# dcmlr/groundgrid

Measured on AMD Instinct MI355X. Metric: point clouds/s (Velodyne-64, ~120k pts, 120m/0.33m grid), higher is better.
Workload: dtype f32+f64 (the reference's mixed float/double arithmetic, bit-exact)

## Files before the change

groundgrid_amd/csrc/gg_context.hip:

```cpp
#include <float.h>
#include <math.h>
#include <stdio.h>
#include <string.h>

#include <algorithm>
#include <atomic>
#include <condition_variable>
#include <cstdlib>
#include <cstdio>
#include <functional>
#include <mutex>
#include <string>
#include <thread>
#include <tuple>
#include <vector>
#include <chrono>

#include <dlfcn.h>
#include <sched.h>
#include <unistd.h>

#include "gg_internal.h"
#include "arena_layout.h"
#include "hip_owned.h"
#include "host_helper.h"
#include "plane_args.h"
#include "region_args.h"
#include "scroll_core.h"
#include "sweep_core.h"

using namespace gg;

namespace {

constexpr int EXPORT_VARIANT_DEFAULT = 0;
constexpr int IMPORT_VARIANT_DEFAULT = 0;
constexpr int IMAGES_VARIANT_DEFAULT = 0;
constexpr int K_SCORE = GG_NUM_KERNELS;

struct EventPair {
    hipEvent_t start, stop;
    int kernel;
    bool owns_start;
};

struct ParamRing {
    Event done[PARAM_RING], done2[PARAM_RING];
    bool used[PARAM_RING]{}, used2[PARAM_RING]{};
    int next = 0;
    hipError_t create()
    {
        hipError_t e = hipSuccess;
        for (int i = 0; i < PARAM_RING && e == hipSuccess; ++i) e = done[i].create();
        for (int i = 0; i < PARAM_RING && e == hipSuccess; ++i) e = done2[i].create();
        return e;
    }
    hipError_t acquire(int *g)
    {
        *g = next;
        next = (next + 1) % PARAM_RING;
        hipError_t e = used[*g] ? hipEventSynchronize(done[*g]) : hipSuccess;
        if (e == hipSuccess && used2[*g]) e = hipEventSynchronize(done2[*g]);
        if (e == hipSuccess) used[*g] = used2[*g] = false;
        return e;
    }
    hipError_t recorded(int g, hipStream_t st)
    {
        const hipError_t e = hipEventRecord(done[g], st);
        if (e == hipSuccess) used[g] = true;
        return e;
    }
    hipError_t recorded2(int g, hipStream_t half_stream)
    {
        const hipError_t e = hipEventRecord(done2[g], half_stream);
        if (e == hipSuccess) used2[g] = true;
        return e;
    }
};

struct CallScratch {
    DeviceBlock<char> dev;
    PinnedBlock<char> pinned;
};

struct RingPart {
    size_t dev, pinned, per_entry;
};
template <typename T>
struct RingTable {
    T *host = nullptr, *dev = nullptr;
    size_t per_entry = 0;
    void bind(const CallScratch &m, const RingPart &p)
    {
        host = (T *)(m.pinned + p.pinned);
        dev = (T *)(m.dev + p.dev);
        per_entry = p.per_entry;
// ... 520 lines not shown
    {
        StageRange stage("interpolation");
        sweep::Params sp = ctx->sweep_params;
        sp.decrease = ctx->cfg.occupied_cells_decrease_factor;
        sp.inv_decrease = 1.0 / sp.decrease;
        sp.decay_fast = sp.decrease >= 1.25 && sp.decrease < 1e300;
        launch_sweep(a, sp, dp, nb, s, ctx->d_sweep_dbg);
    }
    prof.end();
    {
        StageRange stage("segmentation");
        prof.begin(GG_K_LABEL);
        launch_label(a, dp, io, nb, max_n, s);
        prof.end();
        if (score) {
            prof.begin(K_SCORE);
            launch_score(a, dp, io, ctx->score, nb, max_n, s);
            prof.end();
        }
    }
    if (side) hipStreamWaitEvent(s, ctx->join_event, 0);
}

void drop_graphs(gg_context *ctx)
{
    for (auto &e : ctx->graphs) {
        if (e.exec) hipGraphExecDestroy(e.exec);
        if (e.graph) hipGraphDestroy(e.graph);
    }
    ctx->graphs.clear();
}

int launch_or_replay(gg_context *ctx, const Arena &a, const CloudParams *hp, CloudParams *dp, const BatchIO &io, int nb, int max_n, hipStream_t s, const LayerPlan *plan,
                     bool score)
{
    const bool profile = (ctx->flags & GG_FLAG_PROFILE) != 0;
    const bool eligible = nb == 1 && !plan && ctx->graphs_enabled && !profile && !ctx->d_sweep_dbg && s != nullptr && !a.k2_debug && !a.k3_debug && !a.k5_debug && !a.k2_skip;
    if (!eligible) {
        HIPCHK(ctx, hipMemcpyAsync(dp, hp, sizeof(CloudParams) * nb, hipMemcpyHostToDevice, s));
        launch_sequence(ctx, a, dp, io, nb, max_n, s, plan, hp[0].slot, profile, score);
        return GG_OK;
    }
    gg_context::GraphKey key;
    memset(&key, 0, sizeof key);
    key.io = io;
    key.max_n = (int)std::min(ctx->max_points, io.cloud_stride);
    key.slot = hp[0].slot;
    key.flags = a.flags;
    key.eigen = a.eigen_reduction;
    key.generation = ctx->graph_generation;
    key.stream = s;
    if (plan) {
        key.layer_mask = plan->mask & EARLY_LAYERS;
        for (int l = 0; l < GG_NUM_LAYERS; ++l) key.layer_dst[l] = ((key.layer_mask >> l) & 1u) ? plan->dst[l] : nullptr;
    }
    gg_context::GraphEntry *entry = nullptr;
    for (auto &e : ctx->graphs)
        if (memcmp(&e.key, &key, sizeof key) == 0) entry = &e;
    if (!entry) {
        if (ctx->graphs.size() >= 8) {
            size_t victim = 0;
            for (size_t k = 1; k < ctx->graphs.size(); ++k)
                if (ctx->graphs[k].last_use < ctx->graphs[victim].last_use) victim = k;
            if (ctx->graphs[victim].exec) hipGraphExecDestroy(ctx->graphs[victim].exec);
            if (ctx->graphs[victim].graph) hipGraphDestroy(ctx->graphs[victim].graph);
            ctx->graphs.erase(ctx->graphs.begin() + (long)victim);
        }
        ctx->graphs.emplace_back();
        entry = &ctx->graphs.back();
        entry->key = key;
    }
    entry->last_use = ++ctx->graph_clock;
// ... 58 lines not shown
{
    const bool lazy = (ctx->flags & GG_FLAG_MINIMAL_LAYERS) || (batch_entry && !(ctx->flags & GG_FLAG_EAGER_LAYERS));
    const unsigned eff_flags = lazy ? (ctx->flags | GG_FLAG_MINIMAL_LAYERS) : (ctx->flags & ~(unsigned)GG_FLAG_MINIMAL_LAYERS);
    const int nb = b->n_clouds;
    if (nb == 0) return GG_OK;
    int g;
    HIPCHK(ctx, ctx->ring.acquire(&g));
    CloudParams *hp = ctx->h_params + (size_t)g * ctx->n_slots;
    CloudParams *dp = ctx->d_params + (size_t)g * ctx->n_slots;
    int n_first = nb;
    const bool split_wanted = halves_enabled(ctx) && !plan && nb >= ctx->halves_min_clouds && s != ctx->half_stream && s != nullptr;
    if (split_wanted) {
        n_first = 0;
        for (int i = 0; i < nb; ++i) n_first += second_half_slot(ctx, slot_of(b->slots, b->first_slot, i)) ? 0 : 1;
    }
    const bool split = split_wanted && n_first > 0 && n_first < nb;
    if (!split) n_first = nb;
    int max_n[2] = {0, 0}, at[2] = {0, n_first};
    for (int i = 0; i < nb; ++i) {
        const int slot = slot_of(b->slots, b->first_slot, i);
        const int half = split && second_half_slot(ctx, slot) ? 1 : 0;
        CloudParams &p = hp[at[half]++];
        p.slot = slot;
        p.n_points = b->n_points[i];
        p.ox = b->origins[i * 3 + 0];
        p.oy = b->origins[i * 3 + 1];
        p.oz = b->origins[i * 3 + 2];
        p.base_z = (float)b->base_z[i];
        p.pos_x = ctx->pos_x[slot];
        p.pos_y = ctx->pos_y[slot];
        p.has_tf = b->transforms ? 1 : 0;
        p.no_confidence = ctx->no_confidence[slot] ? 1 : 0;
        p.fresh = 0;
        ctx->no_confidence[slot] = 0;
        for (int k = 0; k < 12; ++k) p.tf[k] = b->transforms ? b->transforms[(size_t)i * 12 + k] : 0.0;
        p.label_shift = nb == 1 ? ctx->next_label_shift : 0;
        p.io_index = i;
        p.cfg_index = ctx->slot_own[slot] ? slot : -1;
        if (!confidences_stay_positive(ctx->slot_own[slot] ? ctx->slot_cfg[slot] : ctx->cfg)) ctx->gp_tainted[slot] = 1;
        max_n[half] = std::max(max_n[half], p.n_points);
        ctx->lazy_pending[slot] = lazy ? 1 : 0;
        if (lazy) ctx->lazy_params[slot] = p;
    }
    bool score_half[2] = {false, false};
    if (ctx->score_n_ids)
        for (int i = 0; i < nb; ++i) score_half[i < n_first ? 0 : 1] |= ctx->score_on[hp[i].slot] != 0;
    const bool own_masks = (score_half[0] || score_half[1]) && !b->d_label_masks;
    bool fresh_half[2] = {false, false};
    for (int h = 0; h < (split ? 2 : 1); ++h) {
        const int lo = h ? n_first : 0, hi = h ? nb : n_first;
        bool all = ctx->fresh_enabled && !plan && !ctx->d_sweep_dbg && sweep_takes_fresh(ctx->arena, ctx->sweep_params, hi - lo);
        for (int i = lo; i < hi && all; ++i) all = ctx->fresh[hp[i].slot] != 0 && !ctx->gp_tainted[hp[i].slot];
        fresh_half[h] = all;
        if (all)
            for (int i = lo; i < hi; ++i) hp[i].fresh = 1, ctx->fresh[hp[i].slot] = 0;
    }
    auto fill_fresh = [&](int lo, int hi, hipStream_t on) -> int {
        for (int i = lo; i < hi;) {
            int e = i + 1;
            while (e < hi && hp[e].slot == hp[e - 1].slot + 1) ++e;
            if (const int rc = make_real(ctx, hp[i].slot, e - i, on)) return rc;
            i = e;
        }
        return GG_OK;
    };
    if (s != ctx->stream && ctx->map_event_pending) HIPCHK(ctx, hipStreamWaitEvent(s, ctx->map_event, 0));
    if (ctx->have_batch_event && ctx->last_batch_stream != s && !ctx->probe_unordered_streams) HIPCHK(ctx, hipStreamWaitEvent(s, ctx->batch_event, 0));
    bool joined = false;
    if (!(split && ctx->last_batch_stream == s)) {
        if (const int rc = stream_waits_for_second_half(ctx, s)) return rc;
        joined = true;
    }
    if (split) {
        gg_context::HalvesRecord now;
        const size_t per = b->cloud_stride;
        const uint8_t *p6[7] = {(const uint8_t *)b->d_labels, (const uint8_t *)b->d_out_index, (const uint8_t *)b->d_out_clouds, (const uint8_t *)b->d_out_counts,
                                (const uint8_t *)b->d_label_masks, (const uint8_t *)b->d_out_pc2, own_masks ? ctx->d_score_masks : nullptr};
        const size_t bytes6[7] = {(size_t)nb * per, (size_t)nb * per * 4, (size_t)nb * per * sizeof(gg_point32), (size_t)nb * 64, (size_t)nb * ((per + 3) / 4), (size_t)nb * per * 18,
                                  (size_t)nb * ((per + 3) / 4)};
        for (int k = 0; k < 7; ++k) now.lo[k] = p6[k], now.hi[k] = p6[k] ? p6[k] + bytes6[k] : nullptr;
        uint64_t h = 1469598103934665603ull;
        for (int i = 0; i < nb; ++i) h = (h ^ (uint64_t)(second_half_slot(ctx, slot_of(b->slots, b->first_slot, i)) ? 2 * i + 1 : 2 * i)) * 1099511628211ull;
        now.map_hash = h ^ (uint64_t)nb;
        bool clash = false;
        for (int r = 0; r < ctx->halves_hist_n && !joined && !clash; ++r) {
            const gg_context::HalvesRecord &o = ctx->halves_hist[r];
            if (o.map_hash == now.map_hash) continue;
            for (int x = 0; x < 7 && !clash; ++x)
// ... 26 lines not shown
    io.cloud_stride = b->cloud_stride;
    io.point_format = b->point_format;
    io.d_labels = b->d_labels;
    io.d_out_index = b->d_out_index;
    io.d_out_clouds = b->d_out_clouds;
    io.d_out_counts = b->d_out_counts;
    io.d_label_masks = b->d_label_masks;
    io.d_out_pc2 = b->d_out_pc2;
    BatchIO io_score = io;
    if (own_masks) io_score.d_label_masks = ctx->d_score_masks;

    Arena a = ctx->arena;
    a.flags = eff_flags;
    a.eigen_reduction = ctx->conv.eigen_reduction;
    a.fresh_launch = 0;
    bool own_half[2] = {false, false};
    for (int i = 0; i < nb; ++i) own_half[i < n_first ? 0 : 1] |= hp[i].cfg_index >= 0;
    a.slot_cfg_launch = own_half[0] ? 1 : 0;
    if (split) {
        if (!ctx->probe_no_fork) {
            HIPCHK(ctx, hipEventRecord(ctx->half_fork, s));
            HIPCHK(ctx, hipStreamWaitEvent(ctx->half_stream, ctx->half_fork, 0));
        }
        Arena a2 = a;
        a2.front_sync = a.front_sync2;
        a2.sweep_sync = a.sweep_sync2;
        a2.sweep_rec_clouds = 0;
        a2.scan_sync = a.scan_sync2;
        a2.slot_cfg_launch = own_half[1] ? 1 : 0;
        a.fresh_launch = fresh_half[0] ? 1 : 0;
        a2.fresh_launch = fresh_half[1] ? 1 : 0;
        if (const int rc = fill_fresh(0, n_first, s)) return rc;
        if (const int rc = fill_fresh(n_first, nb, ctx->half_stream)) return rc;
        HIPCHK(ctx, hipMemcpyAsync(dp, hp, sizeof(CloudParams) * n_first, hipMemcpyHostToDevice, s));
        HIPCHK(ctx, hipMemcpyAsync(dp + n_first, hp + n_first, sizeof(CloudParams) * (nb - n_first), hipMemcpyHostToDevice, ctx->half_stream));
        launch_sequence(ctx, a, dp, score_half[0] ? io_score : io, n_first, max_n[0], s, nullptr, hp[0].slot, false, score_half[0]);
        launch_sequence(ctx, a2, dp + n_first, score_half[1] ? io_score : io, nb - n_first, max_n[1], ctx->half_stream, nullptr, hp[n_first].slot, false, score_half[1]);
        HIPCHK(ctx, hipGetLastError());
        HIPCHK(ctx, ctx->ring.recorded2(g, ctx->half_stream));
        HIPCHK(ctx, hipEventRecord(ctx->half_done, ctx->half_stream));
        ctx->have_half_event = true;
    } else {
        a.fresh_launch = fresh_half[0] ? 1 : 0;
        if (const int rc = fill_fresh(0, nb, s)) return rc;
        if (const int rc = launch_or_replay(ctx, a, hp, dp, score_half[0] ? io_score : io, nb, max_n[0], s, plan, score_half[0])) return rc;
        HIPCHK(ctx, hipGetLastError());
    }
    HIPCHK(ctx, ctx->ring.recorded(g, s));
    HIPCHK(ctx, hipEventRecord(ctx->batch_event, s));
    ctx->last_batch_stream = s;
    ctx->have_batch_event = true;
    if (s != ctx->stream) ctx->map_event_pending = false;
    return GG_OK;
}

struct TableUpload {
    size_t offset;
    const void *src;
    size_t bytes;
};
int alloc_call_scratch(gg_context *ctx, const char *who, hipStream_t st, size_t dev_bytes, size_t pinned_bytes, std::initializer_list<TableUpload> tables, CallScratch *mem,
                       ParamRing *ring)
{
    hipStreamCaptureStatus cs = hipStreamCaptureStatusNone;
    if (hipStreamIsCapturing(st, &cs) == hipSuccess && cs != hipStreamCaptureStatusNone)
        return fail(ctx, GG_ERR_INVALID, who, "the first call allocates its scratch and cannot be captured into a graph");
    (void)hipGetLastError();
    CallScratch m;
    ParamRing r;
    int code = GG_ERR_NOMEM;
    const char *what = "device scratch";
    hipError_t e = m.dev.create(dev_bytes);
    if (e == hipSuccess) {
        what = "pinned parameter ring";
        e = m.pinned.create(pinned_bytes);
    }
    if (e == hipSuccess) code = GG_ERR_HIP;
    if (e == hipSuccess && ring) {
// ... 628 lines not shown
        out12[r * 4 + 3] = pose7[r];
    }
    return GG_OK;
}

int gg_get_size(const gg_context *ctx, int *rows, int *cols)
{
    if (!ctx) return GG_ERR_INVALID;
    if (rows) *rows = ctx->arena.g.rows;
    if (cols) *cols = ctx->arena.g.cols;
    return GG_OK;
}

int gg_get_geometry(const gg_context *ctx, double *resolution, double *length_x, double *length_y)
{
    if (!ctx) return GG_ERR_INVALID;
    if (resolution) *resolution = ctx->arena.g.resolution;
    if (length_x) *length_x = ctx->arena.g.length0;
    if (length_y) *length_y = ctx->arena.g.length1;
    return GG_OK;
}

const char *gg_last_error(const gg_context *ctx) { return ctx ? ctx->last_error.c_str() : "null context"; }

int gg_reset_maps(gg_context *ctx, int first_slot, int n, double pos_x, double pos_y, float odom_z, int persistent_only, void *stream)
{
    if (!ctx) return GG_ERR_INVALID;
    if (n < 0) return fail(ctx, GG_ERR_CAPACITY, "gg_reset_maps: n < 0");
    if (const int rc = check_slot_list(ctx, "gg_reset_maps", n, nullptr, first_slot)) return rc;
    if (n == 0) return GG_OK;
    HIPCHK(ctx, hipSetDevice(ctx->device));
    const hipStream_t st = pick_stream(ctx, stream);
    for (int s = first_slot; s < first_slot + n; ++s) ctx->fresh[s] = 0;
    const int boundary = (ctx->n_slots + 1) / 2;
    const bool split = halves_enabled(ctx) && st != ctx->stream && st != ctx->half_stream && st != nullptr && first_slot < boundary && first_slot + n > boundary;
    if (const int rc = call_follows_context(ctx, st, split)) return rc;
    const Arena &a = ctx->arena;
    for (int s = first_slot; s < first_slot + n; ++s) {
        ctx->no_confidence[s] = 1;
        ctx->pos_x[s] = pos_x;
        ctx->pos_y[s] = pos_y;
    }
    const float init[GG_NUM_LAYERS] = {0.0f, odom_z, (float)0.0000001, (float)100.0, (float)-100.0, 0.f, 0.f, 0.f, 0.f, 0.f, 0.f};
    auto fill = [&](int first, int count, hipStream_t on) {
        if (count <= 0) return;
        if (!persistent_only) {
            for (int s = first; s < first + count; ++s) ctx->lazy_pending[s] = 0;
            launch_fill_percall(a, first, count, init, on);
            launch_fill_bytes((uint8_t *)(a.tile_live + (size_t)first * a.tile_live_stride), (size_t)count * a.tile_live_stride * 4, 0xFF, on);
        }
        if (ctx->fresh_enabled) {
            for (int s = first; s < first + count;) {
                if (!ctx->gp_tainted[s]) {
                    ++s;
                    continue;
                }
                int e = s + 1;
                while (e < first + count && ctx->gp_tainted[e]) ++e;
                launch_fill2_strided(gp2_ptr(a, s), (size_t)a.gpl.elems, a.gp2_stride, e - s, init[GG_LAYER_GROUND], init[GG_LAYER_GROUNDPATCH], a.gp_valid, on);
                for (int k = s; k < e; ++k) ctx->gp_tainted[k] = 0;
                s = e;
            }
            launch_reset_fresh(a, first, count, init[GG_LAYER_GROUND], init[GG_LAYER_GROUNDPATCH], on);
            for (int s = first; s < first + count; ++s) ctx->fresh[s] = 1, ctx->fresh_z[s] = odom_z;
        } else {
            launch_fill2_strided(gp2_ptr(a, first), (size_t)a.gpl.elems, a.gp2_stride, count, init[GG_LAYER_GROUND], init[GG_LAYER_GROUNDPATCH], a.gp_valid, on);
            for (int s = first; s < first + count; ++s) ctx->gp_tainted[s] = 0;
        }
    };
    if (split) {
        if (!ctx->probe_no_fork) {
            HIPCHK(ctx, hipEventRecord(ctx->half_fork, st));
            HIPCHK(ctx, hipStreamWaitEvent(ctx->half_stream, ctx->half_fork, 0));
        }
        fill(first_slot, boundary - first_slot, st);
        fill(boundary, first_slot + n - boundary, ctx->half_stream);
        HIPCHK(ctx, hipGetLastError());
        HIPCHK(ctx, hipEventRecord(ctx->half_done, ctx->half_stream));
        ctx->have_half_event = true;
    } else {
        fill(first_slot, n, st);
        HIPCHK(ctx, hipGetLastError());
    }
    return call_recorded(ctx, st, false);
}

int gg_reset_map(gg_context *ctx, int slot, double pos_x, double pos_y, float odom_z)
{
    if (!slot_ok(ctx, slot)) return GG_ERR_CAPACITY;
    return gg_reset_maps(ctx, slot, 1, pos_x, pos_y, odom_z, 0, nullptr);
}

int gg_set_map_position(gg_context *ctx, int slot, double pos_x, double pos_y)
{
    if (!slot_ok(ctx, slot)) return GG_ERR_CAPACITY;
    ctx->pos_x[slot] = pos_x;
// ... 2304 lines not shown
```

groundgrid_amd/csrc/gg_internal.h:

```cpp
#pragma once

#include <hip/hip_runtime.h>
#include <stdint.h>

#include <atomic>
#include <mutex>

#include "groundgrid_hip.h"
#include "gp_layout.h"

namespace gg {

constexpr int TILE = 16;
constexpr int TILE_CELLS = TILE * TILE;
constexpr uint32_t KEY_OUTSIDE = 0xFFFFFFFFu;
constexpr int K2_DBG_WGS = 32768;
constexpr int PW_BIG_CONTEXT_SLOTS = 128;
constexpr int SWEEP_LATENCY_MAX_CLOUDS = 256;
constexpr int K2_MIN_GROUPS_PER_CLOUD = 64;
constexpr int PACKED_TILE_COUNTERS_MIN_T = 1024;
constexpr int K2_LIGHT_MAX = 512;
constexpr int KEY_TILE_SHIFT = 12;
constexpr int SCAN_MAX_PARTS = 16, SCAN_SYNC_WORDS = 1 + SCAN_MAX_PARTS;
constexpr uint32_t KEY_EMIT_BIT = 1u << 10;
// ... 11 lines not shown
    double min_outlier_detection_ground_confidence;
    double distance_factor_sq;
    double minimum_distance_factor_sq;
    double minimum_distance_factor_x10_sq;
    double min_dist_fac;
    double min_point_height_thres;
    double min_point_height_obs_thres;
    double inv_decrease;
    int decay_fast;
};

struct Geometry {
    int rows, cols;
    int C;
    int tiles_r, tiles_c, T;
    double resolution;
    double inv_resolution;
    double length0, length1;
    double half0, half1;
    float resolution_f;
    float min_dist_squared;
    int center;
};

struct CloudParams {
    int slot;
    int n_points;
    float ox, oy, oz;
    float base_z;
    double pos_x, pos_y;
    int has_tf;
    int fresh;
    int no_confidence;
    double tf[12];
    int label_shift;
    int io_index;
    int cfg_index = -1;
};

struct Arena {
    Geometry g;
    DevConfig cfg;
    const float *expected;
    const float4 *patch_table;
    const uint16_t *tile_rank;
    const uint16_t *rank_tile;
    const uint32_t *rank_cell0;
    float *layers;  size_t slot_layer_stride;
    const uint32_t *gp_valid;
    float2 *gp2;    size_t gp2_stride;    GpLayout gpl;
    unsigned long long *gp_bits;  size_t gp_bits_stride;  int gp_fresh_cell;
    int gp_bits_off, gp_bits_words;
    const int *gp_border;  int gp_border_n;
    int gp_border_patched;
    int fresh_launch;
    uint2 *rec;     uint2 *sorted;  size_t point_stride;
    float *zcell;   size_t zcell_stride;
    uint32_t *hist;        size_t hist_stride;
    int hist_pitch;
    uint32_t *front_sync;
    uint32_t *dev_error;
    uint32_t *chunk_emit;  size_t emit_stride;
    uint32_t *totals;
    uint32_t *tile_start;  size_t tile_start_stride;
    uint32_t *tile_live;   size_t tile_live_stride;
    uint4 *tile_list;      size_t tile_list_stride;
    uint32_t *tile_list_cnt;
    unsigned long long *scan_sync;
    uint32_t *front_sync2, *sweep_sync2;
    unsigned long long *scan_sync2;
    uint32_t *sweep_sync;
// ... 466 lines not shown
void launch_match(const MatchArgs &x, int n_maps, hipStream_t s);
void launch_footprint(const FootprintArgs &x, int n_maps, hipStream_t s);
void launch_headings(const HeadingsArgs &x, int n_maps, hipStream_t s);
void launch_tracks(const TrackArgs &x, int n_maps, hipStream_t s);
void launch_boxes(const Arena &a, const BoxArgs &x, int n_clouds, hipStream_t s);
void launch_rollouts(const RolloutArgs &x, int n_maps, hipStream_t s);
void launch_planes_gather(const Arena &a, const PlaneArgs &x, int n_maps, hipStream_t s);
void launch_planes_scatter(const Arena &a, const PlaneArgs &x, int n_maps, hipStream_t s);
void launch_materialise_maps(const Arena &a, const ExportMap *maps, int n_maps, hipStream_t s);
void launch_patch(const Arena &a, const CloudParams *d_params, int n_clouds, hipStream_t s);
void launch_patch_stage(const Arena &a, const CloudParams *d_params, int slot, int section, hipStream_t s);
void launch_stage_cell(const Arena &a, int slot, int stage, int i, int j, hipStream_t s);
namespace sweep {
struct Params;
Params make_params(int n, double resolution, float min_dist_squared, double decrease);
}
void launch_sweep(const Arena &a, const sweep::Params &P, const CloudParams *d_params, int n_clouds, hipStream_t s,
                  unsigned long long *dbg = nullptr);
bool launch_sweep_pair(const Arena &a, const sweep::Params &P, const CloudParams *d_params, int n_clouds, hipStream_t s);
bool sweep_takes_fresh(const Arena &a, const sweep::Params &P, int n_clouds);
bool launch_sweep_pair_batch(const Arena &a, const sweep::Params &P, const CloudParams *d_params, int n_clouds, hipStream_t s);
size_t sweep_pair_rec_floats(const sweep::Params &P);
constexpr int SWEEP_PAIR_MAX_CLOUDS = 16;
size_t sweep_lds_bytes(const sweep::Params &P);
size_t sweep_xchg_entries(const sweep::Params &P);
void launch_label(const Arena &a, const CloudParams *d_params, const BatchIO &io, int n_clouds, int max_n, hipStream_t s);
void launch_score(const Arena &a, const CloudParams *d_params, const BatchIO &io, const ScoreArgs &sc, int n_clouds, int max_n, hipStream_t s);
void launch_fill(float *dst, size_t n, float v, hipStream_t s);
void launch_fill_bytes(uint8_t *dst, size_t n, uint8_t v, hipStream_t s);
void launch_fill_strided(float *dst, size_t n, size_t stride, int count, float v, hipStream_t s);
void launch_fill_percall(const Arena &a, int first_slot, int n_slots, const float init[GG_NUM_LAYERS], hipStream_t s);
void launch_fill2_strided(float2 *dst, size_t n, size_t stride, int count, float x, float y, const uint32_t *valid, hipStream_t s);
void launch_fill2(float2 *dst, size_t n, float x, float y, hipStream_t s);
void launch_reset_fresh(const Arena &a, int first_slot, int count, float x, float y, hipStream_t s);
void launch_layer_to_u8(const float *layer, int rows, int cols, float *d_bounds, uint8_t *d_img, hipStream_t s);
void launch_terrain_image(const Arena &a, int slot, float *d_img, hipStream_t s);
void launch_scroll(const Arena &a, int slot, float2 *scratch, int s0, int s1, double pos_x, double pos_y, const double plane[4], hipStream_t s);
struct MoveParams;
void launch_scroll_batch(const Arena &a, const int2 *cells, const MoveParams *d_params, int n_maps, float2 *scratch, hipStream_t s);
void launch_pack16(const gg_point32 *src, gg_point16 *dst, size_t n, hipStream_t s);
void launch_decode_classes(const Arena &a, int slot, size_t n, uint8_t *d_class, int32_t *d_cell, hipStream_t s);

}
```

groundgrid_amd/csrc/k1_classify.hip:

```cpp
#include "gg_device.h"
#include "sort_core.h"

#include <algorithm>

namespace gg {

constexpr int WALK_MAX_STEP = 1 << 16;
constexpr int WALK_PACKED_MAX = 12;

struct PointIn {
    float x, y, z;
    int ring;
};

template <int FMT>
GG_DEV PointIn load_point(const void *base, size_t idx)
{
    PointIn p;
    if (FMT == GG_POINT16) {
        const uint4 v = reinterpret_cast<const uint4 *>(base)[idx];
        p.x = __uint_as_float(v.x);
        p.y = __uint_as_float(v.y);
        p.z = __uint_as_float(v.z);
        p.ring = (int)(v.w & 0xFFFFu);
// ... 422 lines not shown
__global__ __launch_bounds__(256) void k_fill2_strided(float2 *dst, size_t n, size_t stride, float x, float y, const uint32_t *__restrict__ valid)
{
    constexpr int MAXW = 1024;
    __shared__ uint32_t m[MAXW];
    float2 *d = dst + (size_t)blockIdx.y * stride;
    const size_t words = (n + 31) / 32, per_block = (words + gridDim.x - 1) / gridDim.x;
    for (size_t w0 = (size_t)blockIdx.x * per_block; w0 < min(words, ((size_t)blockIdx.x + 1) * per_block); w0 += MAXW) {
        const size_t nw = min((size_t)MAXW, min(words, ((size_t)blockIdx.x + 1) * per_block) - w0);
        __syncthreads();
        for (size_t k = threadIdx.x; k < nw; k += blockDim.x) m[k] = valid[w0 + k];
        __syncthreads();
        for (size_t p = threadIdx.x; p < nw * 16; p += blockDim.x) {
            const size_t i = (w0 << 5) + 2 * p;
            const uint32_t b = (m[p >> 4] >> ((2 * p) & 31)) & 3u;
            if (b == 3u) {
                typedef float f4_native __attribute__((ext_vector_type(4)));
                const f4_native v4 = {x, y, x, y};
                __builtin_nontemporal_store(v4, reinterpret_cast<f4_native *>(d + i));
            }
            else if (b == 1u)
                d[i] = make_float2(x, y);
            else if (b == 2u)
                d[i + 1] = make_float2(x, y);
        }
    }
}
void launch_fill2_strided(float2 *dst, size_t n, size_t stride, int count, float x, float y, const uint32_t *valid, hipStream_t s)
{
    if (n == 0 || count <= 0) return;
    const int blocks = (int)std::min<size_t>((n + 255) / 256, count >= 64 ? (size_t)32 : (size_t)256);
    hipLaunchKernelGGL(k_fill2_strided, dim3(blocks, count), dim3(256), 0, s, dst, n, stride, x, y, valid);
}

__global__ __launch_bounds__(256) void k_reset_fresh(const Arena a, int first_slot, int count, float x, float y)
{
    const int k = (int)(blockIdx.x * blockDim.x + threadIdx.x);
    if (k < count) gp2_ptr(a, first_slot + k)[a.gp_fresh_cell] = make_float2(x, y);
}
void launch_reset_fresh(const Arena &a, int first_slot, int count, float x, float y, hipStream_t s)
{
    if (count <= 0) return;
    hipLaunchKernelGGL(k_reset_fresh, dim3((count + 255) / 256), dim3(256), 0, s, a, first_slot, count, x, y);
}

__global__ void k_fill_bytes(uint8_t *dst, size_t n, uint8_t v)
{
    for (size_t i = blockIdx.x * (size_t)blockDim.x + threadIdx.x; i < n; i += (size_t)gridDim.x * blockDim.x) dst[i] = v;
}
void launch_fill_bytes(uint8_t *dst, size_t n, uint8_t v, hipStream_t s)
{
    if (n == 0) return;
    const int blocks = (int)std::min<size_t>((n + 255) / 256, (size_t)256);
    hipLaunchKernelGGL(k_fill_bytes, dim3(blocks), dim3(256), 0, s, dst, n, v);
}

void launch_fill(float *dst, size_t n, float v, hipStream_t s)
{
    if (n == 0) return;
    const int blocks = (int)std::min<size_t>((n + 255) / 256, (size_t)2048);
    hipLaunchKernelGGL(k_fill, dim3(blocks), dim3(256), 0, s, dst, n, v);
}

__global__ void k_pack16(const gg_point32 *__restrict__ src, gg_point16 *__restrict__ dst, size_t n)
{
    for (size_t i = blockIdx.x * (size_t)blockDim.x + threadIdx.x; i < n; i += (size_t)gridDim.x * blockDim.x) {
        const PointIn p = load_point<GG_POINT32>(src, i);
        uint4 o;
        o.x = __float_as_uint(p.x);
        o.y = __float_as_uint(p.y);
        o.z = __float_as_uint(p.z);
        o.w = (uint32_t)p.ring;
        reinterpret_cast<uint4 *>(dst)[i] = o;
    }
}

void launch_pack16(const gg_point32 *src, gg_point16 *dst, size_t n, hipStream_t s)
{
// ... 31 lines not shown
```

groundgrid_amd/csrc/k3_patch.hip:

```cpp
#include "gg_device.h"

#include <float.h>

#include <algorithm>

namespace gg {

constexpr int PR = 32, PC = 8, HALO = 2;
constexpr int LR = PR + 2 * HALO, LC = PC + 2 * HALO;

struct PatchCarry {
    bool live;
    int gidx;
    float2 old;
    float pointsblockSum, expected, localmin, maxVar, groundlevel, varThresholdsq;
    int S;
};

GG_DEV void group_fence() { __asm__ volatile("" ::: "memory"); }

template <class F> GG_DEV float stream_tree9(F get)
{
    const float x0 = get(0), x1 = get(1), x2 = get(2), x3 = get(3);
    const float l = (x0 + x1) + (x2 + x3);
// ... 110 lines not shown
    for (int k = tid; k < tiles_c; k += 256) col_has_points[k] = 0u;
    __syncthreads();
    {
        const uint32_t *tile_start = a.tile_start + (size_t)cp.slot * a.tile_start_stride;
        const int tr_lo = (r0 - HALO) / TILE, tr_hi = min((r0 + PR + HALO - 1) / TILE, a.g.tiles_r - 1);
        const int ntr = tr_hi - tr_lo + 1;
        const uint32_t *tile_live = a.tile_live + (size_t)cp.slot * a.tile_live_stride;
        for (int k = tid; k < 3 * tiles_c; k += 256) live_cols[k / tiles_c][k % tiles_c] = 0u;
        __syncthreads();
        for (int k = tid; k < ntr * tiles_c; k += 256) {
            const int tc = k / ntr, tile = (tr_lo + k % ntr) + tc * a.g.tiles_r;
            const int rank = a.tile_rank[tile];
            if (STAGE || tile_start[rank + 1] != tile_start[rank]) col_has_points[tc] = 1u;
            band_rank[k % ntr][tc] = (uint16_t)rank;
            live_cols[k % ntr][tc] = tile_live[rank];
        }
    }
    __syncthreads();
    if (GG_DEBUG_SWITCH(a, k3_debug) == 1) return;
    auto block_has_points = [&](int b) {
        const int tc_lo = (PC * b) / TILE, tc_hi = min((PC * b + LC - 1) / TILE, tiles_c - 1);
        return (col_has_points[tc_lo] | col_has_points[tc_hi]) != 0u;
    };
    auto next_block = [&](int b) {
        while (b < n_blocks && !block_has_points(b)) ++b;
        return b;
    };

    const float *L = percall_ptr(a, cp.slot);
    const float *gp_pts = L + percall_index(0, PL_POINTS, 0);
    const float *gp_var = L + percall_index(0, PL_VARIANCE, 0);
    const float *gp_min = L + percall_index(0, PL_MINGROUNDHEIGHT, 0);
    float2 *gp2 = gp2_ptr(a, cp.slot);
    const uint32_t tag = (!STAGE && cp.fresh != 0) ? 0x80000000u : 0u;

    constexpr int QR = LR / 4;
    static_assert(LR % 4 == 0 && TILE % 4 == 0, "row quads must not straddle half columns");
    float4 sp4 = make_float4(0.f, 0.f, 0.f, 0.f), sv4 = sp4, sm4 = sp4;
    float4 cell_next = make_float4(0.0f, __builtin_inff(), 0.0f, 0.0f);
    const int tr = tid % PR, tcl = tid / PR;
    const int i = r0 + tr;
    const int q_lc = tid / QR, q_lr = 4 * (tid % QR);
    auto request = [&](int b, int first_col, int n_cols) {
        {
            const int jj = HALO + PC * b + tcl;
            const bool v = i < rows && jj < cols && (!STAGE || (i >= bounds.x && i < bounds.y && jj >= bounds.z && jj < bounds.w));
            const float4 e = a.patch_table[v ? (size_t)i + (size_t)jj * rows : (size_t)0];
            float thr_y = e.y, var_z = e.z;
            if (SC && own_thresholds) {
                const bool visited = i >= 2 && jj >= 2 && !(i >= 2 * (cols / 2) - 2 || jj >= rows - 2);
                const double di = (double)i - (double)rows / 2.0, dj = (double)jj - (double)cols / 2.0;
                const float sqdist = (float)((di * di + dj * dj) * res2);
                const bool near = (double)sqdist <= cfg.patch_size_change_distance_sq;
                const double S = near ? 3.0 : 5.0;
                const double thr = std_max(floor(cfg.gpd_min_point_count_threshold * S * (double)e.x), 3.0);
                const float thr_f = (float)thr;
                thr_y = !visited || !(thr < 16777216.0) ? __builtin_inff() : (near ? -thr_f : thr_f);
                var_z = (float)std_min(std_max((double)sqdist * cfg.distance_factor_sq, cfg.minimum_distance_factor_sq), cfg.minimum_distance_factor_x10_sq);
            }
            cell_next = make_float4(e.x, v ? thr_y : __builtin_inff(), var_z, e.w);
        }
        const int gr = r0 - HALO + q_lr, gcol = first_col + q_lc;
        const bool ok = q_lc < n_cols && gr < rows && gcol < cols;
        const int btr = ok ? q_lr / TILE : 0, btc = ok ? gcol / TILE : 0;
        const int cell_in_tile = (gr % TILE) + (gcol % TILE) * TILE;
        const bool live = ok && ((live_cols[btr][btc] >> live_bit(cell_in_tile)) & 1u) != 0u;
        const size_t idx = live ? percall_index((int)band_rank[btr][btc], 0, cell_in_tile) : (size_t)0;
// ... 32 lines not shown
        __syncthreads();
        detect_ground_patch_b(cfg, consume, gp2, tag);
        consume.live = false;

        const int base = (PC * b) & (RING - 1);
        const int lr = tr + HALO, lc = tcl + HALO;
        const bool near = cell_const.y < 0.0f;
        const float threshold = fabsf(cell_const.y);
        if (tid < LC * (PR / 2)) {
            const int c = tid / (PR / 2), r = 2 * (tid % (PR / 2));
            const float *col = pts[base + c] + r;
            const float x0 = col[0], x1 = col[1], x2 = col[2], x3 = col[3], x4 = col[4], x5 = col[5];
            const float mid0 = (x1 + x2) + x3, mid1 = (x2 + x3) + x4;
            v3[c][r] = mid0;
            v5[c][r] = (x0 + x4) + mid0;
            v3[c][r + 1] = mid1;
            v5[c][r + 1] = (x1 + x5) + mid1;
        }
        __syncthreads();
        float pointsblockSum = near ? (v3[tcl + 1][tr] + v3[tcl + 2][tr]) + v3[tcl + 3][tr]
                                    : ((v5[tcl][tr] + v5[tcl + 1][tr]) + (v5[tcl + 2][tr] + v5[tcl + 3][tr])) + v5[tcl + 4][tr];
        if (STAGE) {
            const float(*w)[LR] = pts + base;
            if (near)
                pointsblockSum = stream_tree9([&](int s) { return w[lc - 1 + s / 3][lr - 1 + s % 3]; });
            else if (a.eigen_reduction == GG_EIGEN_34_SSE)
                pointsblockSum = stream_tree25_eigen34([&](int s) { return w[lc - 2 + s / 5][lr - 2 + s % 5]; });
            else
                pointsblockSum = stream_tree25([&](int s) { return w[lc - 2 + s / 5][lr - 2 + s % 5]; });
        }
        const int S = near ? 3 : 5;
        const bool pass = !(pointsblockSum < threshold) && GG_DEBUG_SWITCH(a, k3_debug) != 3;
        produce.gidx = pass ? __float_as_int(cell_const.w) : 0;
        produce.old = gp2[(cp.fresh != 0 && !STAGE) ? a.gp_fresh_cell : produce.gidx];
        produce.live = pass;
        produce.S = S;
        produce.pointsblockSum = pointsblockSum;
        produce.expected = cell_const.x;
        produce.varThresholdsq = cell_const.z;
        group_fence();
        if (pass) {
            if (near)
                patch_sums<3>(a, cfg, pts + base, var + base, mnl + base, lr, lc, produce);
            else
                patch_sums<5>(a, cfg, pts + base, var + base, mnl + base, lr, lc, produce);
        }
        if (nb != b + 1) __syncthreads();
        b = nb;
    };
    PatchCarry c0, c1;
    c0.live = c1.live = false;
    while (b < n_blocks) {
        if (GG_DEBUG_SWITCH(a, k3_debug) == 2) return;
        block_step(c0, c1);
        if (b >= n_blocks) break;
        block_step(c1, c0);
    }
    detect_ground_patch_b(cfg, c0, gp2, tag);
    detect_ground_patch_b(cfg, c1, gp2, tag);
}

void launch_patch(const Arena &a, const CloudParams *d_params, int n_clouds, hipStream_t s)
{
    if (n_clouds == 0) return;
    const int ir = a.g.rows - 2 * HALO, ic = a.g.cols - 2 * HALO;
    if (ir <= 0 || ic <= 0 || a.g.tiles_c > MAXTC) return;
    const int n_bands = (ir + PR - 1) / PR, n_blocks = (ic + PC - 1) / PC;
// ... 42 lines not shown
```

groundgrid_amd/csrc/k4_sweep.hip:

```cpp
#include "gg_device.h"
#include "sweep_core.h"

#include <algorithm>
#include <cstdlib>

#include <stdlib.h>

namespace gg {

using namespace sweep;

typedef uint32_t u32x2 __attribute__((ext_vector_type(2)));

typedef __attribute__((address_space(3))) int lds_int;
typedef __attribute__((address_space(3))) uint64_t lds_u64;

__shared__ __attribute__((aligned(16))) uint32_t sweep_static[4];
#define sweep_wait_failed sweep_static[2]
#define sweep_border_word sweep_static[3]
constexpr uint32_t BORDER_TAGS = 0x10000u;

template <bool DBG> struct DevMemT {
    __amdgpu_buffer_rsrc_t rsrc;
    lds_int *lds;
// ... 519 lines not shown
    Params P_own;
    if (SC) {
        P_own = P_arg;
        DevConfig c;
        load_cloud_config(a, cp.cfg_index, c);
        P_own.decrease = c.occupied_cells_decrease_factor;
        P_own.inv_decrease = c.inv_decrease;
        P_own.decay_fast = c.decay_fast;
    }
    const Params &P = SC ? P_own : P_arg;
    float2 *gp2 = gp2_ptr(a, cp.slot);
    float *percall = percall_ptr(a, cp.slot);
    const int nthreads = blockDim.x;

    for (int k = threadIdx.x; k < L.corner; k += nthreads) lds[k] = 0;
    if (PARTS && threadIdx.x == 0) sweep_wait_failed = 0u;
    const WP centre{1.0f, 1.0f * cp.base_z};
    if (threadIdx.x == 0) {
        if (part == 0) gp2[gp_index(P.gl, P.c, P.c)] = make_float2(cp.base_z, 1.0f);
        float *f = reinterpret_cast<float *>(lds);
        for (int side = 0; side < 2; ++side) {
            f[L.corner + 2 * ((side * P.c + 0) * 2) + 2] = centre.w;
            f[L.corner + 2 * ((side * P.c + 0) * 2) + 3] = centre.p;
        }
        for (int side = SIDE_C; side <= SIDE_D; ++side) {
            f[L.join + 2 * (side * P.c + 0)] = centre.w;
            f[L.join + 2 * (side * P.c + 0) + 1] = centre.p;
        }
    }
    Cell reset{0.f, 0.f};
    bool border_tags = false;
    const bool border_mine = FRESH && a.gp_border_patched && g1 >= P_arg.groups;
    if (FRESH) {
        const float2 init = gp2[a.gp_fresh_cell];
        reset = Cell{__uint_as_float(__builtin_amdgcn_readfirstlane(__float_as_uint(init.x))), __uint_as_float(__builtin_amdgcn_readfirstlane(__float_as_uint(init.y)))};
        if (threadIdx.x == 0) sweep_border_word = 0u;
        if (!a.gp_border_patched) {
            for (int k = (int)threadIdx.x + part * nthreads; k < a.gp_border_n; k += nthreads * n_parts) gp2[a.gp_border[k]] = init;
        } else if (border_mine) {
            bool mine = false;
            for (int k = (int)threadIdx.x; k < a.gp_border_n; k += nthreads) {
                const int e = a.gp_border[k];
                const bool tagged = (int)__float_as_uint(gp2[e].y) < 0;
                if (!tagged) gp2[e] = init;
                mine |= tagged;
            }
            border_tags = __any(mine) != 0;
        }
    }
    if (!P.keep_points) {
        const uint32_t *tile_live = a.tile_live + (size_t)cp.slot * a.tile_live_stride;
        const int lane_ = threadIdx.x & 63, wave_ = (int)(threadIdx.x >> 6) + part * (nthreads >> 6), nwaves = (nthreads >> 6) * n_parts;
        for (int rank = wave_; rank < a.g.T; rank += nwaves) {
            const uint32_t cols_live = tile_live[rank];
            if (!cols_live) continue;
            float *points = percall + percall_index(rank, PL_POINTS, 0);
#pragma unroll
            for (int k = 0; k < 4; ++k) {
                const int cell = lane_ + 64 * k;
                if ((cols_live >> live_bit(cell)) & 1u) points[cell] = 0.0f;
            }
        }
    }
    __syncthreads();
    if (FRESH && border_tags && (threadIdx.x & 63u) == 0u) __hip_atomic_fetch_or(&sweep_border_word, BORDER_TAGS, __ATOMIC_RELAXED, __HIP_MEMORY_SCOPE_WORKGROUP);

    DevMemT<DBG> mem;
// ... 163 lines not shown
```

Measured before the change: 228,300.

## Carry fresh-map reset values in cloud params and upload params on copy stream

The fresh-map reset value (ground height, confidence) moves from a device cell written by a small reset kernel into two fields of the per-cloud parameter record, so the reset kernel launch is dropped and map resets for persistent slots become host-only bookkeeping. Kernels K3 and K4 read the pair from the parameters instead of global memory. For batches larger than the pair limit, the parameter upload is also issued early on a separate H2D stream, and the compute streams wait on an event. This adds event bookkeeping to the parameter ring and relies on the record keeping its size via padding.

```diff
diff --git a/groundgrid_amd/csrc/gg_context.hip b/groundgrid_amd/csrc/gg_context.hip
--- a/groundgrid_amd/csrc/gg_context.hip
+++ b/groundgrid_amd/csrc/gg_context.hip
@@ -45,14 +45,15 @@
 };
 
 struct ParamRing {
-    Event done[PARAM_RING], done2[PARAM_RING];
-    bool used[PARAM_RING]{}, used2[PARAM_RING]{};
+    Event done[PARAM_RING], done2[PARAM_RING], up[PARAM_RING];
+    bool used[PARAM_RING]{}, used2[PARAM_RING]{}, used_up[PARAM_RING]{};
     int next = 0;
     hipError_t create()
     {
         hipError_t e = hipSuccess;
         for (int i = 0; i < PARAM_RING && e == hipSuccess; ++i) e = done[i].create();
         for (int i = 0; i < PARAM_RING && e == hipSuccess; ++i) e = done2[i].create();
+        for (int i = 0; i < PARAM_RING && e == hipSuccess; ++i) e = up[i].create();
         return e;
     }
     hipError_t acquire(int *g)
@@ -61,7 +62,14 @@
         next = (next + 1) % PARAM_RING;
         hipError_t e = used[*g] ? hipEventSynchronize(done[*g]) : hipSuccess;
         if (e == hipSuccess && used2[*g]) e = hipEventSynchronize(done2[*g]);
-        if (e == hipSuccess) used[*g] = used2[*g] = false;
+        if (e == hipSuccess && used_up[*g] && !used[*g]) e = hipEventSynchronize(up[*g]);
+        if (e == hipSuccess) used[*g] = used2[*g] = used_up[*g] = false;
+        return e;
+    }
+    hipError_t uploaded(int g, hipStream_t copy_stream)
+    {
+        const hipError_t e = hipEventRecord(up[g], copy_stream);
+        if (e == hipSuccess) used_up[g] = true;
         return e;
     }
     hipError_t recorded(int g, hipStream_t st)
@@ -648,12 +656,15 @@
 }
 
 int launch_or_replay(gg_context *ctx, const Arena &a, const CloudParams *hp, CloudParams *dp, const BatchIO &io, int nb, int max_n, hipStream_t s, const LayerPlan *plan,
-                     bool score)
+                     bool score, hipEvent_t uploaded)
 {
     const bool profile = (ctx->flags & GG_FLAG_PROFILE) != 0;
     const bool eligible = nb == 1 && !plan && ctx->graphs_enabled && !profile && !ctx->d_sweep_dbg && s != nullptr && !a.k2_debug && !a.k3_debug && !a.k5_debug && !a.k2_skip;
     if (!eligible) {
-        HIPCHK(ctx, hipMemcpyAsync(dp, hp, sizeof(CloudParams) * nb, hipMemcpyHostToDevice, s));
+        if (uploaded)
+            HIPCHK(ctx, hipStreamWaitEvent(s, uploaded, 0));
+        else
+            HIPCHK(ctx, hipMemcpyAsync(dp, hp, sizeof(CloudParams) * nb, hipMemcpyHostToDevice, s));
         launch_sequence(ctx, a, dp, io, nb, max_n, s, plan, hp[0].slot, profile, score);
         return GG_OK;
     }
@@ -778,6 +789,7 @@
         p.has_tf = b->transforms ? 1 : 0;
         p.no_confidence = ctx->no_confidence[slot] ? 1 : 0;
         p.fresh = 0;
+        p.fresh_ground = p.fresh_confidence = 0.0f;
         ctx->no_confidence[slot] = 0;
         for (int k = 0; k < 12; ++k) p.tf[k] = b->transforms ? b->transforms[(size_t)i * 12 + k] : 0.0;
         p.label_shift = nb == 1 ? ctx->next_label_shift : 0;
@@ -799,7 +811,25 @@
         for (int i = lo; i < hi && all; ++i) all = ctx->fresh[hp[i].slot] != 0 && !ctx->gp_tainted[hp[i].slot];
         fresh_half[h] = all;
         if (all)
-            for (int i = lo; i < hi; ++i) hp[i].fresh = 1, ctx->fresh[hp[i].slot] = 0;
+            for (int i = lo; i < hi; ++i) {
+                hp[i].fresh = 1, hp[i].fresh_ground = ctx->fresh_z[hp[i].slot], hp[i].fresh_confidence = (float)0.0000001;
+                ctx->fresh[hp[i].slot] = 0;
+            }
+    }
+    hipEvent_t uploaded = nullptr;
+    if (nb > SWEEP_PAIR_MAX_CLOUDS && !plan) {
+        hipStreamCaptureStatus cs = hipStreamCaptureStatusNone;
+        const bool plain = hipStreamIsCapturing(s, &cs) == hipSuccess && cs == hipStreamCaptureStatusNone;
+        (void)hipGetLastError();
+        if (plain) {
+            HIPCHK(ctx, hipMemcpyAsync(dp, hp, sizeof(CloudParams) * nb, hipMemcpyHostToDevice, ctx->h2d_stream));
+            const hipError_t e = ctx->ring.uploaded(g, ctx->h2d_stream);
+            if (e != hipSuccess) {
+                (void)hipStreamSynchronize(ctx->h2d_stream);
+                return fail(ctx, GG_ERR_HIP, "hipEventRecord behind the parameter upload", e);
+            }
+            uploaded = ctx->ring.up[g];
+        }
     }
     auto fill_fresh = [&](int lo, int hi, hipStream_t on) -> int {
         for (int i = lo; i < hi;) {
@@ -892,8 +922,13 @@
         a2.fresh_launch = fresh_half[1] ? 1 : 0;
         if (const int rc = fill_fresh(0, n_first, s)) return rc;
         if (const int rc = fill_fresh(n_first, nb, ctx->half_stream)) return rc;
-        HIPCHK(ctx, hipMemcpyAsync(dp, hp, sizeof(CloudParams) * n_first, hipMemcpyHostToDevice, s));
-        HIPCHK(ctx, hipMemcpyAsync(dp + n_first, hp + n_first, sizeof(CloudParams) * (nb - n_first), hipMemcpyHostToDevice, ctx->half_stream));
+        if (uploaded) {
+            HIPCHK(ctx, hipStreamWaitEvent(s, uploaded, 0));
+            HIPCHK(ctx, hipStreamWaitEvent(ctx->half_stream, uploaded, 0));
+        } else {
+            HIPCHK(ctx, hipMemcpyAsync(dp, hp, sizeof(CloudParams) * n_first, hipMemcpyHostToDevice, s));
+            HIPCHK(ctx, hipMemcpyAsync(dp + n_first, hp + n_first, sizeof(CloudParams) * (nb - n_first), hipMemcpyHostToDevice, ctx->half_stream));
+        }
         launch_sequence(ctx, a, dp, score_half[0] ? io_score : io, n_first, max_n[0], s, nullptr, hp[0].slot, false, score_half[0]);
         launch_sequence(ctx, a2, dp + n_first, score_half[1] ? io_score : io, nb - n_first, max_n[1], ctx->half_stream, nullptr, hp[n_first].slot, false, score_half[1]);
         HIPCHK(ctx, hipGetLastError());
@@ -903,7 +938,7 @@
     } else {
         a.fresh_launch = fresh_half[0] ? 1 : 0;
         if (const int rc = fill_fresh(0, nb, s)) return rc;
-        if (const int rc = launch_or_replay(ctx, a, hp, dp, score_half[0] ? io_score : io, nb, max_n[0], s, plan, score_half[0])) return rc;
+        if (const int rc = launch_or_replay(ctx, a, hp, dp, score_half[0] ? io_score : io, nb, max_n[0], s, plan, score_half[0], uploaded)) return rc;
         HIPCHK(ctx, hipGetLastError());
     }
     HIPCHK(ctx, ctx->ring.recorded(g, s));
@@ -1598,6 +1633,17 @@
     HIPCHK(ctx, hipSetDevice(ctx->device));
     const hipStream_t st = pick_stream(ctx, stream);
     for (int s = first_slot; s < first_slot + n; ++s) ctx->fresh[s] = 0;
+    bool host_only = persistent_only && ctx->fresh_enabled;
+    for (int s = first_slot; s < first_slot + n && host_only; ++s) host_only = !ctx->gp_tainted[s];
+    if (host_only) {
+        for (int s = first_slot; s < first_slot + n; ++s) {
+            ctx->no_confidence[s] = 1;
+            ctx->pos_x[s] = pos_x;
+            ctx->pos_y[s] = pos_y;
+            ctx->fresh[s] = 1, ctx->fresh_z[s] = odom_z;
+        }
+        return GG_OK;
+    }
     const int boundary = (ctx->n_slots + 1) / 2;
     const bool split = halves_enabled(ctx) && st != ctx->stream && st != ctx->half_stream && st != nullptr && first_slot < boundary && first_slot + n > boundary;
     if (const int rc = call_follows_context(ctx, st, split)) return rc;
@@ -1627,7 +1673,6 @@
                 for (int k = s; k < e; ++k) ctx->gp_tainted[k] = 0;
                 s = e;
             }
-            launch_reset_fresh(a, first, count, init[GG_LAYER_GROUND], init[GG_LAYER_GROUNDPATCH], on);
             for (int s = first; s < first + count; ++s) ctx->fresh[s] = 1, ctx->fresh_z[s] = odom_z;
         } else {
             launch_fill2_strided(gp2_ptr(a, first), (size_t)a.gpl.elems, a.gp2_stride, count, init[GG_LAYER_GROUND], init[GG_LAYER_GROUNDPATCH], a.gp_valid, on);
diff --git a/groundgrid_amd/csrc/gg_internal.h b/groundgrid_amd/csrc/gg_internal.h
--- a/groundgrid_amd/csrc/gg_internal.h
+++ b/groundgrid_amd/csrc/gg_internal.h
@@ -67,11 +67,14 @@
     int has_tf;
     int fresh;
     int no_confidence;
+    float fresh_ground;
     double tf[12];
     int label_shift;
     int io_index;
     int cfg_index = -1;
-};
+    float fresh_confidence;
+};
+static_assert(sizeof(CloudParams) == 168, "the reset's pair of a fresh map fits into the record's padding");
 
 struct Arena {
     Geometry g;
@@ -604,7 +607,6 @@
 void launch_fill_percall(const Arena &a, int first_slot, int n_slots, const float init[GG_NUM_LAYERS], hipStream_t s);
 void launch_fill2_strided(float2 *dst, size_t n, size_t stride, int count, float x, float y, const uint32_t *valid, hipStream_t s);
 void launch_fill2(float2 *dst, size_t n, float x, float y, hipStream_t s);
-void launch_reset_fresh(const Arena &a, int first_slot, int count, float x, float y, hipStream_t s);
 void launch_layer_to_u8(const float *layer, int rows, int cols, float *d_bounds, uint8_t *d_img, hipStream_t s);
 void launch_terrain_image(const Arena &a, int slot, float *d_img, hipStream_t s);
 void launch_scroll(const Arena &a, int slot, float2 *scratch, int s0, int s1, double pos_x, double pos_y, const double plane[4], hipStream_t s);
diff --git a/groundgrid_amd/csrc/k1_classify.hip b/groundgrid_amd/csrc/k1_classify.hip
--- a/groundgrid_amd/csrc/k1_classify.hip
+++ b/groundgrid_amd/csrc/k1_classify.hip
@@ -478,17 +478,6 @@
     hipLaunchKernelGGL(k_fill2_strided, dim3(blocks, count), dim3(256), 0, s, dst, n, stride, x, y, valid);
 }
 
-__global__ __launch_bounds__(256) void k_reset_fresh(const Arena a, int first_slot, int count, float x, float y)
-{
-    const int k = (int)(blockIdx.x * blockDim.x + threadIdx.x);
-    if (k < count) gp2_ptr(a, first_slot + k)[a.gp_fresh_cell] = make_float2(x, y);
-}
-void launch_reset_fresh(const Arena &a, int first_slot, int count, float x, float y, hipStream_t s)
-{
-    if (count <= 0) return;
-    hipLaunchKernelGGL(k_reset_fresh, dim3((count + 255) / 256), dim3(256), 0, s, a, first_slot, count, x, y);
-}
-
 __global__ void k_fill_bytes(uint8_t *dst, size_t n, uint8_t v)
 {
     for (size_t i = blockIdx.x * (size_t)blockDim.x + threadIdx.x; i < n; i += (size_t)gridDim.x * blockDim.x) dst[i] = v;
diff --git a/groundgrid_amd/csrc/k3_patch.hip b/groundgrid_amd/csrc/k3_patch.hip
--- a/groundgrid_amd/csrc/k3_patch.hip
+++ b/groundgrid_amd/csrc/k3_patch.hip
@@ -166,7 +166,9 @@
     const float *gp_var = L + percall_index(0, PL_VARIANCE, 0);
     const float *gp_min = L + percall_index(0, PL_MINGROUNDHEIGHT, 0);
     float2 *gp2 = gp2_ptr(a, cp.slot);
-    const uint32_t tag = (!STAGE && cp.fresh != 0) ? 0x80000000u : 0u;
+    const bool fresh_cloud = !STAGE && cp.fresh != 0;
+    const uint32_t tag = fresh_cloud ? 0x80000000u : 0u;
+    const float2 fresh_pair = make_float2(cp.fresh_ground, cp.fresh_confidence);
 
     constexpr int QR = LR / 4;
     static_assert(LR % 4 == 0 && TILE % 4 == 0, "row quads must not straddle half columns");
@@ -265,7 +267,8 @@
         const int S = near ? 3 : 5;
         const bool pass = !(pointsblockSum < threshold) && GG_DEBUG_SWITCH(a, k3_debug) != 3;
         produce.gidx = pass ? __float_as_int(cell_const.w) : 0;
-        produce.old = gp2[(cp.fresh != 0 && !STAGE) ? a.gp_fresh_cell : produce.gidx];
+        const float2 old_mem = gp2[fresh_cloud ? 0 : produce.gidx];
+        produce.old = fresh_cloud ? fresh_pair : old_mem;
         produce.live = pass;
         produce.S = S;
         produce.pointsblockSum = pointsblockSum;
diff --git a/groundgrid_amd/csrc/k4_sweep.hip b/groundgrid_amd/csrc/k4_sweep.hip
--- a/groundgrid_amd/csrc/k4_sweep.hip
+++ b/groundgrid_amd/csrc/k4_sweep.hip
@@ -575,7 +575,7 @@
     bool border_tags = false;
     const bool border_mine = FRESH && a.gp_border_patched && g1 >= P_arg.groups;
     if (FRESH) {
-        const float2 init = gp2[a.gp_fresh_cell];
+        const float2 init = make_float2(cp.fresh_ground, cp.fresh_confidence);
         reset = Cell{__uint_as_float(__builtin_amdgcn_readfirstlane(__float_as_uint(init.x))), __uint_as_float(__builtin_amdgcn_readfirstlane(__float_as_uint(init.y)))};
         if (threadIdx.x == 0) sweep_border_word = 0u;
         if (!a.gp_border_patched) {
```

Result: no change. 228,300, median of 4 (+0.0%).
